# ExaScience/bpmf

Hardware: AMD Instinct MI355X
Metric: user+item column samples/sec per Gibbs iter; test RMSE vs reference (higher is better)
Workload: dtype f64

## Files before the change

bpmf_amd/csrc/kernels.h:

```cpp
#pragma once
#include <hip/hip_runtime.h>
#include <stdint.h>

#include "philox.h"
#include "args.h"

namespace bpmf {

typedef double d4 __attribute__((ext_vector_type(4)));

__device__ __forceinline__ d4 mfma16(double a, double b, d4 c)
{
    return __builtin_amdgcn_mfma_f64_16x16x4f64(a, b, c, 0, 0, 0);
}

__device__ __forceinline__ double mfma44(double a, double b, double c)
{
    return __builtin_amdgcn_mfma_f64_4x4x4f64(a, b, c, 0, 0, 0);
}

template <int K>
struct Rot44 {
    static constexpr int NT = K / 16;
    __host__ __device__ static constexpr int nrot(int TI, int TJ) { return TI == TJ ? 3 : 4; }
// ... 18 lines not shown
    const int lo = __builtin_amdgcn_update_dpp(0, (int)v, CTRL, 0xF, 0xF, true);
    const int hi = __builtin_amdgcn_update_dpp(0, (int)(v >> 32), CTRL, 0xF, 0xF, true);
    return __builtin_bit_cast(double, ((long long)hi << 32) | (unsigned int)lo);
}

template <int K>
__device__ __forceinline__ void rot44_contract(const double (&yy)[K / 16], double (&C)[Rot44<K>::NACC])
{
    using G = Rot44<K>;
    constexpr int NT = K / 16;
    double rot[NT][3];
#pragma unroll
    for (int t = 0; t < NT; ++t) {
        rot[t][0] = yy[t];
        rot[t][1] = quad_rot<1>(yy[t]);
        rot[t][2] = quad_rot<2>(yy[t]);
    }
#pragma unroll
    for (int TI = 0; TI < NT; ++TI)
#pragma unroll
        for (int TJ = TI; TJ < NT; ++TJ)
#pragma unroll
            for (int d = 0; d < G::nrot(TI, TJ); ++d) {
                if (d < 3) C[G::aoff(TI, TJ) + d] = mfma44(yy[TI], rot[TJ][d], C[G::aoff(TI, TJ) + d]);
                else C[G::aoff(TI, TJ) + d] = mfma44(rot[TI][1], yy[TJ], C[G::aoff(TI, TJ) + d]);
            }
}

template <int K, typename Sink>
__device__ __forceinline__ void rot44_images(const double (&C)[Rot44<K>::NACC], double *buf0, double *buf1, int lane, Sink &&sink)
{
    using G = Rot44<K>;
    constexpr int NT = G::NT;
    const int i = lane >> 4, b = (lane >> 2) & 3, j = lane & 3;
    int tix = 0;
#pragma unroll
    for (int TI = 0; TI < NT; ++TI)
#pragma unroll
        for (int TJ = TI; TJ < NT; ++TJ, ++tix) {
            double *img = (tix & 1) ? buf1 : buf0;
#pragma unroll
            for (int d = 0; d < G::nrot(TI, TJ); ++d) {
                const int row = d < 3 ? 4 * b + i : 4 * ((b + 1) & 3) + i, col = d < 3 ? 4 * ((b + d) & 3) + j : 4 * b + j;
                const double v = C[G::aoff(TI, TJ) + d];
                img[row * 16 + col] = v;
                if (TI == TJ && d > 0) img[col * 16 + row] = v;
            }
            __syncthreads();
#pragma unroll
            for (int m = 0; m < 4; ++m) sink(tix, TI, TJ, m, img[(4 * m + i) * 16 + (lane & 15)]);
            __syncthreads();
        }
}

__device__ __forceinline__ double rsqrt_nr(double d)
{
    const double y0 = __builtin_amdgcn_rsq(d);
    const double e = fma(-d, y0 * y0, 1.0);
    const double q = e * fma(0.375, e, 0.5);
    return fma(y0, q, y0);
}

__device__ __forceinline__ double gbcast(double v, int base_bytes, int off)
{
    const int lo = __builtin_amdgcn_ds_bpermute(base_bytes + 4 * off, __double2loint(v));
    const int hi = __builtin_amdgcn_ds_bpermute(base_bytes + 4 * off, __double2hiint(v));
    return __hiloint2double(hi, lo);
}

__device__ __forceinline__ double bcast(double v, int src)
{
    const int lo = __builtin_amdgcn_readlane(__double2loint(v), src);
    const int hi = __builtin_amdgcn_readlane(__double2hiint(v), src);
    return __hiloint2double(hi, lo);
}


__device__ __forceinline__ double polar_r2(double x, double y)
{
#pragma clang fp contract(off)
    return x * x + y * y;
}

__device__ __forceinline__ uint32_t sample_counter(int64_t idx, int ktrue, uint32_t iter_plus_1)
{
    return (uint32_t)((uint64_t)(idx + 1) * (uint64_t)ktrue * (uint64_t)iter_plus_1);
}

#define BPMF_RLX_SYSTEM_ __ATOMIC_RELAXED, __HIP_MEMORY_SCOPE_SYSTEM
enum { BPMF_TMO_GATE = 1, BPMF_TMO_PARAMS = 2, BPMF_TMO_STATS = 3 };
__device__ __forceinline__ void flag_timeout(unsigned long long *tmo, unsigned long long what)
{
    if (tmo) __hip_atomic_store(tmo, what, BPMF_RLX_SYSTEM_);
}

__device__ __forceinline__ void wait_params(const SampleArgs &a)
{
    if (a.gate_flag == nullptr) return;
    const unsigned long long t0 = wall_clock64();
    const unsigned long long limit = a.wait_ticks + (a.wait_ticks >> 1);
    while ((unsigned)__builtin_amdgcn_readfirstlane((int)__hip_atomic_load(a.gate_flag, __ATOMIC_RELAXED, __HIP_MEMORY_SCOPE_AGENT)) != a.gate_want) {
        __builtin_amdgcn_s_sleep(8);
        if (wall_clock64() - t0 > limit) {
            if (threadIdx.x == 0) flag_timeout(a.tmo, BPMF_TMO_PARAMS);
            break;
        }
    }
    asm volatile("" ::: "memory");
}

#ifndef BPMF_PROFILING
#define BPMF_PROFILING 0
#endif
constexpr bool kProfiling = BPMF_PROFILING != 0;
__device__ __forceinline__ uint32_t ablate_bits(const SampleArgs &a)
{
    if constexpr (kProfiling) return a.ablate;
    else return 0u;
}

__device__ __forceinline__ void stamp(const SampleArgs &a, int w, int slot)
{
    if constexpr (!kProfiling) {
        __builtin_amdgcn_sched_barrier(0);
        return;
    }
    if (a.stamps == nullptr || threadIdx.x != 0) return;
    const int probe = (w == 0) ? 0 : ((w == a.nwork / 2) ? 1 : -1);
    if (probe >= 0 && slot < 64) a.stamps[probe * 64 + slot] = wall_clock64();
}

__device__ __forceinline__ int rank_below(unsigned long long m)
{
    return (int)__builtin_amdgcn_mbcnt_hi((unsigned)(m >> 32), __builtin_amdgcn_mbcnt_lo((unsigned)m, 0u));
}

template <int NMAX>
__device__ __forceinline__ void draw_normals(uint32_t counter, int n, double *out_lds, int lane, int pad_to = 0)
{
    for (int i = n + lane; i < pad_to; i += 64) out_lds[i] = 0.0;
    int produced = 0;
    uint32_t base = 0;
    while (produced < n) {
        const Philox4 b = stream_block(counter, base + (uint32_t)lane);
        const double x = 2.0 * canonical53(b.w[3], b.w[2]) - 1.0;
        const double y = 2.0 * canonical53(b.w[1], b.w[0]) - 1.0;
        const double r2 = polar_r2(x, y);
        const bool acc = !(r2 > 1.0 || r2 == 0.0);
        const unsigned long long m = __ballot(acc);
        const int rank = produced + rank_below(m);
        if (acc && rank < n) {
            out_lds[rank] = y * polar_mult(r2);
        }
        produced += __popcll(m);
        base += 64u;
    }
}

template <int NMAX>
__device__ __forceinline__ void draw_normals_deferred(uint32_t counter, int n, double *out_lds, double *r2_lds, int lane, int pad_to = 0)
{
    for (int i = n + lane; i < pad_to; i += 64) out_lds[i] = 0.0;
    int produced = 0;
    uint32_t base = 0;
    while (produced < n) {
        const Philox4 b = stream_block(counter, base + (uint32_t)lane);
        const double x = 2.0 * canonical53(b.w[3], b.w[2]) - 1.0;
        const double y = 2.0 * canonical53(b.w[1], b.w[0]) - 1.0;
        const double r2 = polar_r2(x, y);
        const bool acc = !(r2 > 1.0 || r2 == 0.0);
        const unsigned long long m = __ballot(acc);
        const int rank = produced + rank_below(m);
        if (acc && rank < n) { out_lds[rank] = y; r2_lds[rank] = r2; }
        produced += __popcll(m);
        base += 64u;
    }
    for (int i = lane; i < n; i += 64) {
        const double r2 = r2_lds[i];
        out_lds[i] = out_lds[i] * polar_mult(r2);
    }
}

template <int NMAX>
__device__ __forceinline__ void draw_normals_pair(uint32_t counterA, uint32_t counterB, int n, double *outA, double *outB,
                                                  double *r2A, double *r2B, int lane, int pad_to = 0)
{
    for (int i = n + lane; i < pad_to; i += 64) { outA[i] = 0.0; outB[i] = 0.0; }
    auto attempt = [&](uint32_t counter, uint32_t block, double &y, double &r2) -> bool {
        const Philox4 b = stream_block(counter, block);
        const double x = 2.0 * canonical53(b.w[3], b.w[2]) - 1.0;
        y = 2.0 * canonical53(b.w[1], b.w[0]) - 1.0;
        r2 = polar_r2(x, y);
        return !(r2 > 1.0 || r2 == 0.0);
    };
    int prodA, prodB;
    {
        double y, r2;
        bool acc = attempt(counterA, (uint32_t)lane, y, r2);
        unsigned long long m = __ballot(acc);
        int rank = rank_below(m);
        if (acc && rank < n) { outA[rank] = y; r2A[rank] = r2; }
        prodA = __popcll(m);
        acc = attempt(counterB, (uint32_t)lane, y, r2);
        m = __ballot(acc);
        rank = rank_below(m);
        if (acc && rank < n) { outB[rank] = y; r2B[rank] = r2; }
        prodB = __popcll(m);
    }
    const bool hi = lane >= 32;
    const int l32 = lane & 31;
    uint32_t base = 64u;
    while (prodA < n || prodB < n) {
        double y, r2;
        const bool acc = attempt(hi ? counterB : counterA, base + (uint32_t)l32, y, r2);
        const unsigned long long m = __ballot(acc);
        const unsigned mA = (unsigned)m, mB = (unsigned)(m >> 32);
        const int rank = hi ? prodB + (int)__builtin_amdgcn_mbcnt_hi(mB, 0u) : prodA + (int)__builtin_amdgcn_mbcnt_lo(mA, 0u);
        if (acc && rank < n) { (hi ? outB : outA)[rank] = y; (hi ? r2B : r2A)[rank] = r2; }
        prodA += __popc(mA); prodB += __popc(mB);
        base += 32u;
    }
    for (int i = lane; i < n; i += 64) {
        const double ra = r2A[i], rb = r2B[i];
        outA[i] = outA[i] * polar_mult(ra);
        outB[i] = outB[i] * polar_mult(rb);
    }
}

template <int K>
__device__ __forceinline__ void gram_chunk(const int32_t *__restrict__ rowidx, const double *__restrict__ vals, int len,
                                           const double *__restrict__ other, const double *__restrict__ zero_row, double mean, double alpha,
                                           d4 (&acc)[Geo<K>::NTRI], double (&r)[Geo<K>::NT], int lane, int rowmask = -1)
{
    constexpr int NT = Geo<K>::NT;
    const int kq = lane >> 4, li = lane & 15;
    int ri_n = (0 + lane < len) ? rowidx[lane] : -1;
    double wv_n = (0 + lane < len) ? (vals[lane] - mean) * alpha : 0.0;
    for (int b = 0; b < len; b += 64) {
        const int ri = ri_n;
        const double wv = wv_n;
        if (b + 64 < len) {
            const int q = b + 64 + lane;
            ri_n = (q < len) ? rowidx[q] : -1;
            wv_n = (q < len) ? (vals[q] - mean) * alpha : 0.0;
        }
        const int nsteps = (len - b >= 64) ? 16 : (len - b + 3) >> 2;
        double y[4][NT], w[4];
        auto gather = [&](int g, double (&yy)[4][NT], double (&ww)[4]) {
#pragma unroll
            for (int s = 0; s < 4; ++s) {
                const int src = (g * 4 + s) * 4 + kq;
                const int row = __shfl(ri, src);
                ww[s] = __shfl(wv, src);
                const double *col = (row >= 0) ? other + (size_t)(row & rowmask) * K : zero_row;
#pragma unroll
                for (int t = 0; t < NT; ++t) yy[s][t] = col[(t * 16 + li < K) ? t * 16 + li : 0];
            }
        };
        gather(0, y, w);
#pragma unroll
        for (int g = 0; g < 4; ++g) {
            if (g * 4 >= nsteps) break;
            double yn[4][NT], wn[4];
            const bool more = (g + 1) * 4 < nsteps;
            if (g < 3 && more) gather(g + 1, yn, wn);
#pragma unroll
            for (int s = 0; s < 4; ++s) {
#pragma unroll
                for (int t = 0; t < NT; ++t) r[t] = fma(y[s][t], w[s], r[t]);
                int tri = 0;
#pragma unroll
                for (int I = 0; I < NT; ++I)
#pragma unroll
                    for (int J = I; J < NT; ++J, ++tri) acc[tri] = mfma16(y[s][I], y[s][J], acc[tri]);
            }
            if (g < 3 && more) {
#pragma unroll
                for (int s = 0; s < 4; ++s) {
                    w[s] = wn[s];
#pragma unroll
                    for (int t = 0; t < NT; ++t) y[s][t] = yn[s][t];
                }
            }
        }
    }
#pragma unroll
    for (int t = 0; t < NT; ++t) {
        r[t] += __shfl_xor(r[t], 16);
        r[t] += __shfl_xor(r[t], 32);
    }
}

template <int CTRL>
__device__ __forceinline__ double row_ror_add(double x)
{
    const long long v = __builtin_bit_cast(long long, x);
    const int lo = (int)v, hi = (int)(v >> 32);
    const int rlo = __builtin_amdgcn_update_dpp(0, lo, CTRL, 0xF, 0xF, true);
    const int rhi = __builtin_amdgcn_update_dpp(0, hi, CTRL, 0xF, 0xF, true);
    const long long rv = ((long long)rhi << 32) | (unsigned int)rlo;
    return x + __builtin_bit_cast(double, rv);
}

template <bool WT> struct IdxBlockT { int ri; double v; int base; };
template <> struct IdxBlockT<true> { int ri; double v; int base; double s; };
typedef IdxBlockT<false> IdxBlock;
template <bool WT = false>
__device__ __forceinline__ IdxBlockT<WT> load_idx_block(const int32_t *__restrict__ rowidx, const double *__restrict__ vals, int base, int lane, int len,
                                                        const double *__restrict__ safe, const double *__restrict__ sw = nullptr)
{
    IdxBlockT<WT> r;
    const int q = base + lane;
    const int32_t *pr = (q < len) ? rowidx + q : reinterpret_cast<const int32_t *>(safe);
    const double *pv = (q < len) ? vals + q : safe;
    r.ri = *pr;
    r.v = *pv;
    if constexpr (WT) {
        const double *ps = (q < len) ? sw + q : safe;
        r.s = *ps;
    }
    r.base = base;
    return r;
}

template <int K, bool WT = false>
__device__ __forceinline__ void gram_chunk44(const int32_t *__restrict__ rowidx, const double *__restrict__ vals, int len,
                                             const double *__restrict__ other, const double *__restrict__ zero_row,
                                             double mean, double alpha, IdxBlockT<WT> cur, IdxBlockT<WT> nxt,
                                             double (&acc)[Geo44<K>::NB], double (&rr)[Geo44<K>::NG], int lane, int rowmask = -1,
                                             const double *__restrict__ sw = nullptr)
{
    using G = Geo44<K>;
    constexpr int NG = G::NG, NL = G::NL;
    typedef double dd2 __attribute__((ext_vector_type(2)));
    const int slot = lane >> 2, x = lane & 3;
    auto gather = [&](const IdxBlockT<WT> &ib, int gg, dd2 (&yy)[NL], double &ww, double &ss) {
        const int src = gg * 16 + slot;
        const int row = __shfl(ib.ri, src);
        ww = (__shfl(ib.v, src) - mean) * alpha;
        if constexpr (WT) ss = __shfl(ib.s, src);
        const double *base = (ib.base + src < len) ? other + (size_t)(row & rowmask) * K : zero_row;
        const dd2 *p = reinterpret_cast<const dd2 *>(base + 2 * x);
#pragma unroll
        for (int h = 0; h < NL; ++h) yy[h] = p[4 * h];
    };
    auto contract = [&](const dd2 (&yy)[NL], double ww, double ss) {
        double R[NG];
#pragma unroll
        for (int h = 0; h < NL; ++h) { R[2 * h] = yy[h].x; R[2 * h + 1] = yy[h].y; }
        if constexpr (WT) {
#pragma unroll
            for (int g = 0; g < NG; ++g) R[g] *= ss;
        }
#pragma unroll
        for (int g = 0; g < NG; ++g) rr[g] = fma(R[g], ww, rr[g]);
        int blk = 0;
#pragma unroll
        for (int g = 0; g < NG; ++g)
#pragma unroll
            for (int g2 = g; g2 < NG; ++g2, ++blk) acc[blk] = mfma44(R[g], R[g2], acc[blk]);
    };
    if (len <= 0) return;
    dd2 yA[NL], yB[NL];
    double wA, wB = 0.0, sA = 0.0, sB = 0.0;
    gather(cur, 0, yA, wA, sA);
    int b0 = 0;
    for (; b0 + 64 < len; b0 += 64) {
        IdxBlockT<WT> nn{};
        if constexpr (!WT) nn = load_idx_block<WT>(rowidx, vals, b0 + 128, lane, len, zero_row, sw);
        gather(cur, 1, yB, wB, sB);
        contract(yA, wA, sA);
        gather(cur, 2, yA, wA, sA);
        contract(yB, wB, sB);
        gather(cur, 3, yB, wB, sB);
        contract(yA, wA, sA);
        gather(nxt, 0, yA, wA, sA);
        contract(yB, wB, sB);
        cur = nxt;
        if constexpr (WT) nxt = load_idx_block<WT>(rowidx, vals, b0 + 128, lane, len, zero_row, sw);
        else nxt = nn;
    }
    const int ng = (len - b0 + 15) >> 4;
    if (ng > 1) gather(cur, 1, yB, wB, sB);
    contract(yA, wA, sA);
    if (ng > 1) {
        if (ng > 2) gather(cur, 2, yA, wA, sA);
        contract(yB, wB, sB);
        if (ng > 2) {
            if (ng > 3) gather(cur, 3, yB, wB, sB);
            contract(yA, wA, sA);
            if (ng > 3) contract(yB, wB, sB);
        }
    }
}

typedef double gs_raw __attribute__((ext_vector_type(2)));
__device__ __forceinline__ gs_raw load_gs_rec(const GatherRec *__restrict__ rec, int g, unsigned slot_bytes)
{
    return *reinterpret_cast<const gs_raw *>(reinterpret_cast<const char *>(rec + 16 * g) + slot_bytes);
}

template <int K>
__device__ __forceinline__ void gram_stream44(const GatherRec *__restrict__ rec, int ng, const double *__restrict__ other,
                                              const double *__restrict__ zero_row, double alpha, gs_raw r0, gs_raw r1, unsigned slot_bytes,
                                              double (&acc)[Geo44<K>::NB], double (&rr)[Geo44<K>::NG], int lane)
{
    using G = Geo44<K>;
    constexpr int NG = G::NG, NL = G::NL;
    typedef double dd2 __attribute__((ext_vector_type(2)));
    const int x = lane & 3;
    const dd2 *ox = reinterpret_cast<const dd2 *>(other + 2 * x), *zx = reinterpret_cast<const dd2 *>(zero_row + 2 * x);
    auto gather = [&](const gs_raw &rc, dd2 (&yy)[NL], double &ww) {
        const int off = (int)__builtin_bit_cast(long long, rc.x);
        ww = rc.y * alpha;
        const dd2 *p = (off >= 0) ? ox + off : zx;
#pragma unroll
        for (int h = 0; h < NL; ++h) yy[h] = p[4 * h];
    };
    auto contract = [&](const dd2 (&yy)[NL], double ww) {
        double R[NG];
#pragma unroll
        for (int h = 0; h < NL; ++h) { R[2 * h] = yy[h].x; R[2 * h + 1] = yy[h].y; }
#pragma unroll
        for (int g = 0; g < NG; ++g) rr[g] = fma(R[g], ww, rr[g]);
        int blk = 0;
#pragma unroll
        for (int g = 0; g < NG; ++g)
#pragma unroll
            for (int g2 = g; g2 < NG; ++g2, ++blk) acc[blk] = mfma44(R[g], R[g2], acc[blk]);
    };
    if (ng <= 0) return;
    dd2 yA[NL], yB[NL];
    double wA, wB = 0.0;
    gather(r0, yA, wA);
    r0 = load_gs_rec(rec, 2, slot_bytes);
    if (ng > 1) gather(r1, yB, wB);
    r1 = load_gs_rec(rec, 3, slot_bytes);
    contract(yA, wA);
    int g = 1;
    for (; g + 2 < ng; g += 2) {
        gather(r0, yA, wA);
        r0 = load_gs_rec(rec, g + 3, slot_bytes);
        contract(yB, wB);
        gather(r1, yB, wB);
        r1 = load_gs_rec(rec, g + 4, slot_bytes);
        contract(yA, wA);
    }
    if (g < ng) {
        if (g + 1 < ng) gather(r0, yA, wA);
        contract(yB, wB);
        if (g + 1 < ng) contract(yA, wA);
    }
}

template <int K>
__device__ __forceinline__ void assemble44(double (&acc)[Geo44<K>::NB], double (&rr)[Geo44<K>::NG], double *sA, double *sb,
                                           int LD, int lane)
{
    using G = Geo44<K>;
    constexpr int NG = G::NG;
    static_assert(NG % 2 == 0, "block rows are written in pairs");
    const int i = lane >> 4, b = (lane >> 2) & 3, j = lane & 3;
    auto blk = [](int g, int g2) constexpr { return g * NG - (g * (g - 1)) / 2 + (g2 - g); };
    double *up = sA + (2 * i) * LD + 2 * j;
    double *lo = sA + (2 * j) * LD + 2 * i;
#pragma unroll
    for (int g = 0; g < NG; g += 2) {
#pragma unroll
        for (int t = blk(g, g); t < blk(g + 1, NG - 1) + 1; ++t) {
            const double v = row_ror_add<0x128>(acc[t]);
            acc[t] = row_ror_add<0x124>(v);
        }
        if (b == 0) {
            up[G::idx(g + 1, 0) * LD + G::idx(g + 1, 0)] = acc[blk(g + 1, g + 1)];
#pragma unroll
            for (int g2 = g; g2 < NG; g2 += 2) {
                double2 v; v.x = acc[blk(g, g2)]; v.y = acc[blk(g, g2 + 1)];
                *reinterpret_cast<double2 *>(&up[G::idx(g, 0) * LD + G::idx(g2, 0)]) = v;
                if (g2 > g) {
                    double2 w; w.x = acc[blk(g + 1, g2)]; w.y = acc[blk(g + 1, g2 + 1)];
                    *reinterpret_cast<double2 *>(&up[G::idx(g + 1, 0) * LD + G::idx(g2, 0)]) = w;
                }
            }
        } else if (b == 1) {
            lo[G::idx(g + 1, 0) * LD + G::idx(g, 0)] = acc[blk(g, g + 1)];
#pragma unroll
            for (int g2 = g + 2; g2 < NG; ++g2) {
                double2 v; v.x = acc[blk(g, g2)]; v.y = acc[blk(g + 1, g2)];
                *reinterpret_cast<double2 *>(&lo[G::idx(g2, 0) * LD + G::idx(g, 0)]) = v;
            }
        }
    }
#pragma unroll
    for (int g = 0; g < NG; ++g) {
        double v = row_ror_add<0x128>(rr[g]);
        v = row_ror_add<0x124>(v);
        v += __shfl_xor(v, 16);
        v += __shfl_xor(v, 32);
        if (lane < 4) sb[G::idx(g, lane)] = v;
    }
}

template <int K>
__device__ __forceinline__ void deposit_column(const SampleArgs &a, int64_t idx, const d4 (&acc)[Geo<K>::NTRI],
                                               const double (&r)[Geo<K>::NT], double *lds, int slot, int lane)
{
    using G = Geo<K>;
    constexpr int NT = G::NT;
    const int kq = lane >> 4, li = lane & 15;
    double *sL = lds + slot * G::SLOT, *sY = sL + G::PLEN, *sZ = sY + K;

    draw_normals<K>(sample_counter(idx, a.ktrue, a.iter_plus_1), a.ktrue, sZ, lane, K);
    const double *LF = a.prop_lambda ? a.prop_lambda + (size_t)(idx - a.col_from) * K * K : a.LambdaF;

    int tri = 0;
#pragma unroll
    for (int I = 0; I < NT; ++I)
#pragma unroll
        for (int J = I; J < NT; ++J, ++tri)
#pragma unroll
            for (int reg = 0; reg < 4; ++reg) {
                const int gi = I * 16 + kq + 4 * reg, gj = J * 16 + li;
                const int row = (I == J) ? gi : gj, col = (I == J) ? gj : gi;
                if (row < K && col <= row)
                    sL[tri_off(row) + col] = (a.diag_only && row != col) ? 0.0 : fma(a.alpha, acc[tri][reg], LF[row + col * K]);
            }
    if (kq == 0) {
#pragma unroll
        for (int t = 0; t < NT; ++t)
            if (t * 16 + li < K) {
                double lm = a.Lmu[t * 16 + li];
                if (a.prop_lambda) {
                    lm = 0.0;
                    for (int j = 0; j < K; ++j) lm = fma(LF[t * 16 + li + j * K], a.mu[j], lm);
                }
                sY[t * 16 + li] = lm + r[t];
            }
    }
    if (lane == 0) reinterpret_cast<long long *>(lds + G::C * G::SLOT)[slot] = idx;
}

template <int K>
struct Pivot { double dinv0, dinv1, l10; };

template <int K>
__device__ __forceinline__ Pivot<K> factor_block(double pa, double pb, double pc)
{
    Pivot<K> v;
    v.dinv0 = rsqrt_nr(pa);
    const double rdet = rsqrt_nr(fma(pa, pc, -(pb * pb)));
    v.dinv1 = rdet * (pa * v.dinv0);
    v.l10 = pb * v.dinv0;
    return v;
}

template <int K>
__device__ __forceinline__ void finish_slots(const SampleArgs &a, double *lds, int nfilled, int lane_in)
{
    using G = Geo<K>;
    constexpr int NP = G::NP;
    int lane = lane_in;
    asm volatile("" : "+v"(lane));
    const int c = lane / K, i = lane % K;
    double *sL = lds + c * G::SLOT, *sY = sL + G::PLEN, *sZ = sY + K;
    double *myrow = sL + tri_off(i);
    const int gbase = 4 * (c * K);
    __syncthreads();

    double row[K + 1];
#pragma unroll
    for (int j = 0; j < K; j += 2) {
        const double2 g = *reinterpret_cast<const double2 *>(&myrow[j]);
        row[j] = g.x;
        row[j + 1] = g.y;
    }
    row[K] = sY[i];
    const double zi = sZ[i];
    Pivot<K> pv = factor_block<K>(sL[0], sL[tri_off(1)], sL[tri_off(1) + 1]);
    __syncthreads();

#pragma unroll
    for (int p = 0; p < NP; ++p) {
        const int k = 2 * p;
        double2 lp;
        lp.x = row[k] * pv.dinv0;
        lp.y = fma(-lp.x, pv.l10, row[k + 1]) * pv.dinv1;
        if (i >= k) *reinterpret_cast<double2 *>(&myrow[k]) = lp;

        double na = 0.0, nb = 0.0, nc = 0.0;
        if (p + 1 < NP) {
            na = gbcast(row[k + 2], gbase, k + 2);
            nb = gbcast(row[k + 2], gbase, k + 3);
            nc = gbcast(row[k + 3], gbase, k + 3);
        }
        const double rb0 = gbcast(row[K], gbase, k), rb1 = gbcast(row[K], gbase, k + 1);
        __syncthreads();
        const double2 L = *reinterpret_cast<const double2 *>(&myrow[k]);
        Pivot<K> pn = pv;
        if (p + 1 < NP) {
            const double2 l0 = *reinterpret_cast<const double2 *>(&sL[tri_off(k + 2) + k]);
            const double2 l1 = *reinterpret_cast<const double2 *>(&sL[tri_off(k + 3) + k]);
            const double pa = fma(-l0.y, l0.y, fma(-l0.x, l0.x, na));
            const double pb = fma(-l1.y, l0.y, fma(-l1.x, l0.x, nb));
            const double pc = fma(-l1.y, l1.y, fma(-l1.x, l1.x, nc));
            pn = factor_block<K>(pa, pb, pc);
        }
        const double yk = rb0 * pv.dinv0;
        const double yk1 = fma(-pv.l10, yk, rb1) * pv.dinv1;
        if (i == 0) *reinterpret_cast<double2 *>(&sY[k]) = double2{yk, yk1};
        row[K] = fma(-L.y, yk1, fma(-L.x, yk, row[K]));
#pragma unroll
        for (int j = k + 2; j < K; ++j) {
            const double2 A = *reinterpret_cast<const double2 *>(&sL[tri_off(j) + k]);
            row[j] = fma(-L.y, A.y, fma(-L.x, A.x, row[j]));
        }
#pragma unroll
        for (int m = k + 2; m < K + 1; ++m) asm volatile("" : "+v"(row[m]));
        pv = pn;
    }
    __syncthreads();

    double bi = sY[i] + zi;
    const double my_dinv = 1.0 / myrow[i];
    constexpr int BB = K < 8 ? K : 8;
#pragma unroll
    for (int kb = K - BB; kb >= 0; kb -= BB) {
        double lv[BB];
#pragma unroll
        for (int t = 0; t < BB; ++t) lv[t] = sL[tri_off(kb + t) + i];
#pragma unroll
        for (int t = BB - 1; t >= 0; --t) {
            const int k = kb + t;
            if (k == 0) continue;
            const double xk = gbcast(bi * my_dinv, gbase, k);
            bi = (i < k) ? fma(-lv[t], xk, bi) : bi;
        }
    }
    const double xi = bi * my_dinv;

    if (c < nfilled) {
        const long long idx = reinterpret_cast<const long long *>(lds + G::C * G::SLOT)[c];
        a.items[(size_t)idx * K + i] = xi;
        if (!(fabs(xi) <= 1.79769313486231570815e+308)) atomicMin(a.fail, (unsigned long long)idx);
    }
    __syncthreads();
}

#define BPMF_RLX_AGENT __ATOMIC_RELAXED, __HIP_MEMORY_SCOPE_AGENT

template <int K>
struct Geo1 {
    static constexpr int S = (64 / K < K / 2) ? 64 / K : K / 2;
    static constexpr int NP = K / 2;
    static constexpr int QN = NP / S;
    static constexpr int M = 2 * QN;
    static constexpr int FLD = K + 2;
    static constexpr bool PACKED = K == 64;
    __host__ __device__ static constexpr int roff_c(int j) { return (j & 1) ? ((j + 1) * (j + 1)) / 2 : (j * (j + 2)) / 2; }
    static constexpr int AWORDS = PACKED ? roff_c(K) : K * FLD;
    static constexpr int LANES = K * S;
    static constexpr int LDS_WORDS = AWORDS + 4 * K + 2;
    static constexpr int WPS = K == 32 ? 3 : (K < 32 ? 4 : 2);
};

template <int K, typename Assemble>
__device__ __forceinline__ void finish_single(const SampleArgs &a, int col_local, double *lds, int lane_in, bool have_z,
                                              Assemble &&assemble)
{
    int lane = lane_in;
    using G = Geo1<K>;
    constexpr int LD = G::FLD, S = G::S, NP = G::NP, QN = G::QN, M = G::M;
    asm volatile("" : "+v"(lane));
    double *sA = lds, *sb = lds + G::AWORDS, *sz = sb + K, *sdummy = sz + K, *szero = sdummy + 2 * K;
    auto roff = [](int j) -> int {
        if constexpr (G::PACKED) return (j & 1) ? ((j + 1) * (j + 1)) >> 1 : (j * (j + 2)) >> 1;
        else return j * G::FLD;
    };
    const int64_t idx = a.col_from + col_local;

    if (!have_z) draw_normals<K>(sample_counter(idx, a.ktrue, a.iter_plus_1), a.ktrue, sz, lane, K);

    const int l = lane & (G::LANES - 1);
    const int h = l / K, i = l % K;
    const double *LF = a.prop_lambda ? a.prop_lambda + (size_t)col_local * K * K : a.LambdaF;
    constexpr bool PRELOAD = K <= 32;
    double lf[PRELOAD ? M : 2];
    if constexpr (PRELOAD) {
#pragma unroll
        for (int q = 0; q < QN; ++q) {
            const int j = 2 * (q * S + h);
            lf[2 * q] = LF[i + j * K];
            lf[2 * q + 1] = LF[i + (j + 1) * K];
        }
    }
    double lmu = a.Lmu[i];
    if (a.prop_lambda) {
        lmu = 0.0;
        for (int j = 0; j < K; ++j) lmu = fma(LF[i + j * K], a.mu[j], lmu);
    }

    assemble(sA, sb, LD, lane);
    if (lane < 2) szero[lane] = 0.0;
    __syncthreads();

    double row[M + 2];
#pragma unroll
    for (int q = 0; q < QN; ++q) {
        double2 g;
        if constexpr (G::PACKED) {
            const int j = 2 * (q * S + h);
            g.x = sA[(j <= i) ? roff(i) + j : roff(j) + i];
            g.y = sA[(j + 1 <= i) ? roff(i) + j + 1 : roff(j + 1) + i];
        } else {
            g = *reinterpret_cast<const double2 *>(&sA[i * LD + 2 * (q * S + h)]);
        }
        if constexpr (PRELOAD) {
            row[2 * q] = fma(a.alpha, g.x, lf[2 * q]);
            row[2 * q + 1] = fma(a.alpha, g.y, lf[2 * q + 1]);
        } else {
            const int j = 2 * (q * S + h);
            row[2 * q] = fma(a.alpha, g.x, LF[i + j * K]);
            row[2 * q + 1] = fma(a.alpha, g.y, LF[i + (j + 1) * K]);
        }
    }
    if (a.diag_only) {
#pragma unroll
        for (int q = 0; q < QN; ++q) {
            const int j = 2 * (q * S + h);
            row[2 * q] = (j == i) ? row[2 * q] : 0.0;
            row[2 * q + 1] = (j + 1 == i) ? row[2 * q + 1] : 0.0;
        }
    }
    row[M] = (h == 0) ? lmu + sb[i] : 0.0;
    row[M + 1] = 0.0;
    const double zi = sz[i];
    double yi = 0.0;
    __syncthreads();

#pragma unroll
    for (int p = 0; p < NP; ++p) {
        const int hk = p % S, qk = p / S, k = 2 * p;
        const int src0 = hk * K + k, src1 = src0 + 1;
        const double pa = bcast(row[2 * qk], src0);
        const double pb = bcast(row[2 * qk], src1);
        const double pc = bcast(row[2 * qk + 1], src1);
        const double bk = bcast(row[M], k), bk1 = bcast(row[M], k + 1);
        const double dinv0 = rsqrt_nr(pa);
        const double rdet = rsqrt_nr(fma(pa, pc, -(pb * pb)));
        const double dinv1 = rdet * (pa * dinv0);
        const double l10 = pb * dinv0;
        const double yk = bk * dinv0;
        const double yk1 = fma(-l10, yk, bk1) * dinv1;
        yi = (i == k) ? yk : yi;
        yi = (i == k + 1) ? yk1 : yi;
        double2 lp;
        lp.x = row[2 * qk] * dinv0;
        lp.y = fma(-lp.x, l10, row[2 * qk + 1]) * dinv1;
        double *dst = (h == hk && (!G::PACKED || i >= k)) ? &sA[roff(i) + k] : &sdummy[2 * i];
        *reinterpret_cast<double2 *>(dst) = lp;
        __syncthreads();
        const double2 L = *reinterpret_cast<const double2 *>((!G::PACKED || i >= k) ? &sA[roff(i) + k] : szero);
        row[M] = fma(-L.y, yk1, fma(-L.x, yk, row[M]));
        if constexpr (S > 1) {
            const int j0 = 2 * (qk * S + h);
            const double2 A0 = *reinterpret_cast<const double2 *>(&sA[roff(j0) + k]);
            const double2 A1 = *reinterpret_cast<const double2 *>(&sA[roff(j0 + 1) + k]);
            const double u0 = fma(-L.y, A0.y, fma(-L.x, A0.x, row[2 * qk]));
            const double u1 = fma(-L.y, A1.y, fma(-L.x, A1.x, row[2 * qk + 1]));
            row[2 * qk] = (h > hk) ? u0 : row[2 * qk];
            row[2 * qk + 1] = (h > hk) ? u1 : row[2 * qk + 1];
        }
#pragma unroll
        for (int q = qk + 1; q < QN; ++q) {
            const int j0 = 2 * (q * S + h);
            const double2 A0 = *reinterpret_cast<const double2 *>(&sA[roff(j0) + k]);
            const double2 A1 = *reinterpret_cast<const double2 *>(&sA[roff(j0 + 1) + k]);
            row[2 * q] = fma(-L.y, A0.y, fma(-L.x, A0.x, row[2 * q]));
            row[2 * q + 1] = fma(-L.y, A1.y, fma(-L.x, A1.x, row[2 * q + 1]));
        }
#pragma unroll
        for (int m = 2 * qk; m < M + 1; ++m) asm volatile("" : "+v"(row[m]));
    }

    double bi = yi + zi;
    const double my_dinv = 1.0 / sA[roff(i) + i];
    constexpr int BB = K < 8 ? K : 8;
#pragma unroll
    for (int kb = K - BB; kb >= 0; kb -= BB) {
        double lv[BB];
#pragma unroll
        for (int t = 0; t < BB; ++t) lv[t] = *((i < kb + t) ? &sA[roff(kb + t) + i] : szero);
#pragma unroll
        for (int t = BB - 1; t >= 0; --t) {
            const int k = kb + t;
            if (k == 0) continue;
            const double xk = bcast(bi * my_dinv, k);
            bi = fma(-lv[t], xk, bi);
        }
    }
    const double xi = bi * my_dinv;

    if (lane < K) a.items[(size_t)idx * K + lane] = xi;
    const bool bad = !(fabs(xi) <= 1.79769313486231570815e+308);
    if (__any(bad) && lane == 0) atomicMin(a.fail, (unsigned long long)idx);
}

template <int K>
__device__ __forceinline__ void colstats_body(int w, const double *__restrict__ items, int64_t c0, int64_t c1, int nwaves,
                                              double *partials, const unsigned long long *__restrict__ fail_in,
                                              double *__restrict__ out, unsigned *ticket, unsigned *flag, unsigned seq,
                                              unsigned long long *tmo, unsigned long long wait_ticks, double *img);
__device__ __forceinline__ void gate_stage_body(int block, int nblocks, const unsigned *gate_host, unsigned want, const double *src_host,
                                                double *__restrict__ dst, int n, unsigned *dflag, unsigned dval,
                                                unsigned long long *tmo, unsigned long long wait_ticks);

template <int K, bool GS, bool WT = false>
__device__ __forceinline__ void sample1_body(const SampleArgs &a, const FusedArgs &f, double *lds)
{
    const int lane = threadIdx.x;
    int bid = blockIdx.x;
    if (f.gate_host) {
        if (bid == 0) { gate_stage_body(0, 1, f.gate_host, f.gate_want, f.src_host, f.dst, f.n, f.dflag, f.dval, a.tmo, a.wait_ticks); return; }
        --bid;
    }
    if (bid < f.nstat) {
        colstats_body<K>(bid, f.st_items, f.st_c0, f.st_c1, f.nstat, f.st_partials, f.st_fail, f.st_out, f.st_ticket, f.st_flag, f.st_seq,
                         f.st_tmo, a.wait_ticks, lds);
        return;
    }
    const int w = bid - f.nstat;
    const int col = a.wi_col[w];
    const int64_t p0 = a.wi_p0[w];
    const int len = a.wi_len[w];
    const int mc = a.wi_mc[w];

    const int glen = (ablate_bits(a) & 2u) ? 0 : len;
    static_assert(!(GS && WT), "the gather stream carries no weights");
    IdxBlockT<WT> ib0{}, ib1{};
    gs_raw gr0{}, gr1{};
    const GatherRec *rec = nullptr;
    const unsigned slot_bytes = 16u * ((unsigned)lane >> 2);
    int ng = 0;
    if constexpr (GS) {
        rec = a.gs_rec + (size_t)a.gs_g0[w] * 16;
        ng = (ablate_bits(a) & 2u) ? 0 : a.gs_ng[w];
        gr0 = load_gs_rec(rec, 0, slot_bytes);
        gr1 = load_gs_rec(rec, 1, slot_bytes);
    } else {
        ib0 = load_idx_block<WT>(a.rowidx + p0, a.vals + p0, 0, lane, glen, a.zero_row, WT ? a.sw + p0 : nullptr);
        ib1 = load_idx_block<WT>(a.rowidx + p0, a.vals + p0, 64, lane, glen, a.zero_row, WT ? a.sw + p0 : nullptr);
    }

    if (mc < 0 && !(ablate_bits(a) & 1u))
        draw_normals<K>(sample_counter(a.col_from + col, a.ktrue, a.iter_plus_1), a.ktrue, lds + Geo1<K>::AWORDS + K, lane, K);

    static_assert(K <= 32, "k_sample1: K <= 32 (K = 64 runs the slab form, K = 128 the workgroup form)");
    {
        using G4 = Geo44<K>;
        constexpr int NB = G4::NB, NG = G4::NG, PART = G4::PART;
        double acc[NB], rr[NG];
#pragma unroll
        for (int t = 0; t < NB; ++t) acc[t] = 0.0;
#pragma unroll
        for (int t = 0; t < NG; ++t) rr[t] = 0.0;
        if constexpr (GS)
            gram_stream44<K>(rec, ng, a.other_items, a.zero_row, a.alpha, gr0, gr1, slot_bytes, acc, rr, lane);
        else
            gram_chunk44<K, WT>(a.rowidx + p0, a.vals + p0, glen, a.other_items, a.zero_row, a.mean_rating, a.alpha, ib0, ib1, acc, rr, lane,
                                (ablate_bits(a) & 4u) ? 63 : -1, WT ? a.sw + p0 : nullptr);
        if (ablate_bits(a) & 1u) {
            double v = rr[0];
#pragma unroll
            for (int t = 0; t < NB; ++t) v += acc[t];
            if (mc < 0 && lane < K) a.items[(size_t)(a.col_from + col) * K + lane] = v;
            return;
        }
        if (mc >= 0) {
            const int nch = a.mc_nchunks[mc];
            double *pbase = a.partials + (size_t)a.mc_slot0[mc] * PART;
            double *p = pbase + (size_t)a.wi_chunk[w] * PART;
#pragma unroll
            for (int t = 0; t < NB; ++t) __hip_atomic_store(&p[t * 64 + lane], acc[t], BPMF_RLX_AGENT);
#pragma unroll
            for (int t = 0; t < NG; ++t) __hip_atomic_store(&p[(NB + t) * 64 + lane], rr[t], BPMF_RLX_AGENT);
            asm volatile("s_waitcnt vmcnt(0)" ::: "memory");
            unsigned t = 0;
            if (lane == 0) t = __hip_atomic_fetch_add(&a.mc_count[mc], 1u, BPMF_RLX_AGENT);
            t = __builtin_amdgcn_readfirstlane(t);
            if ((int)t != nch - 1) return;
            if (lane == 0) __hip_atomic_store(&a.mc_count[mc], 0u, BPMF_RLX_AGENT);
#pragma unroll
            for (int t2 = 0; t2 < NB; ++t2) acc[t2] = 0.0;
#pragma unroll
            for (int t2 = 0; t2 < NG; ++t2) rr[t2] = 0.0;
            for (int ch = 0; ch < nch; ++ch) {
                const double *pc = pbase + (size_t)ch * PART;
                double tmp[NB + NG];
#pragma unroll
                for (int t2 = 0; t2 < NB + NG; ++t2) tmp[t2] = __hip_atomic_load(&pc[t2 * 64 + lane], BPMF_RLX_AGENT);
#pragma unroll
                for (int t2 = 0; t2 < NB; ++t2) acc[t2] += tmp[t2];
#pragma unroll
                for (int t2 = 0; t2 < NG; ++t2) rr[t2] += tmp[NB + t2];
            }
        }
        wait_params(a);
        finish_single<K>(a, col, lds, lane, mc < 0,
                         [&](double *sA, double *sb, int LD, int ln) { assemble44<K>(acc, rr, sA, sb, LD, ln); });
    }
}

template <int K>
__global__ __launch_bounds__(64, Geo1<K>::WPS) void k_sample1(SampleArgs a, FusedArgs f)
{
    __shared__ __attribute__((aligned(16))) double lds[Geo1<K>::LDS_WORDS];
    sample1_body<K, true>(a, f, lds);
}

template <int K>
__global__ __launch_bounds__(64, Geo1<K>::WPS) void k_sample1i(SampleArgs a, FusedArgs f)
{
    __shared__ __attribute__((aligned(16))) double lds[Geo1<K>::LDS_WORDS];
    sample1_body<K, false>(a, f, lds);
}

template <int K>
__global__ __launch_bounds__(64, Geo1<K>::WPS) void k_sample1w(SampleArgs a, FusedArgs f)
{
    __shared__ __attribute__((aligned(16))) double lds[Geo1<K>::LDS_WORDS];
    sample1_body<K, false, true>(a, f, lds);
}

#define BPMF_RLX_SYSTEM __ATOMIC_RELAXED, __HIP_MEMORY_SCOPE_SYSTEM
__device__ __forceinline__ void publish_when_last(unsigned *ticket, unsigned nblocks, unsigned *flag_host, unsigned seq,
                                                  unsigned *rearm = nullptr, unsigned *rearm2 = nullptr)
{
    asm volatile("s_waitcnt vmcnt(0)" ::: "memory");
    __syncthreads();
    if (threadIdx.x == 0) {
        const unsigned t = __hip_atomic_fetch_add(ticket, 1u, BPMF_RLX_AGENT);
        if (t == nblocks - 1) {
            __hip_atomic_store(ticket, 0u, BPMF_RLX_AGENT);
            if (rearm) __hip_atomic_store(rearm, 0u, BPMF_RLX_AGENT);
            if (rearm2) __hip_atomic_store(rearm2, 0u, BPMF_RLX_AGENT);
            __hip_atomic_store(flag_host, seq, BPMF_RLX_SYSTEM);
        }
    }
}

template <int K>
constexpr bool kColstatsRot = (K == 64);

template <int K>
__device__ __forceinline__ void colstats_accumulate(const double *__restrict__ items, int64_t b, int64_t e,
                                                    d4 (&acc)[Geo<K>::NTRI], double (&r)[Geo<K>::NT], int lane, double *img,
                                                    const int32_t *__restrict__ list = nullptr, int64_t c0 = 0)
{
    constexpr int NT = Geo<K>::NT;
    constexpr bool ROT = kColstatsRot<K>;
    const int kq = lane >> 4, li = lane & 15;
    double C[ROT ? Rot44<K>::NACC : 1];
#pragma unroll
    for (int t = 0; t < (ROT ? Rot44<K>::NACC : 1); ++t) C[t] = 0.0;
#pragma unroll
    for (int t = 0; t < Geo<K>::NTRI; ++t) acc[t] = d4{0.0, 0.0, 0.0, 0.0};
#pragma unroll
    for (int t = 0; t < NT; ++t) r[t] = 0.0;
    double yn[2][NT];
    int64_t idn[2];
    auto ids = [&](int64_t c, int64_t (&id)[2]) {
#pragma unroll
        for (int s = 0; s < 2; ++s) {
            const int64_t pos = (c + s * 4 + kq < e) ? c + s * 4 + kq : b;
            id[s] = list ? c0 + (int64_t)list[pos] : pos;
        }
    };
    auto fetch = [&](const int64_t (&id)[2], double (&yy)[2][NT]) {
#pragma unroll
        for (int s = 0; s < 2; ++s) {
            const double *x = items + (size_t)id[s] * K;
#pragma unroll
            for (int t = 0; t < NT; ++t) yy[s][t] = x[(t * 16 + li < K) ? t * 16 + li : 0];
        }
    };
    if (b < e) {
        int64_t id0[2];
        ids(b, id0);
        fetch(id0, yn);
        ids((b + 8 < e) ? b + 8 : b, idn);
    }
    for (int64_t c = b; c < e; c += 8) {
        double y[2][NT];
#pragma unroll
        for (int s = 0; s < 2; ++s) {
            const bool ok = c + s * 4 + kq < e;
#pragma unroll
            for (int t = 0; t < NT; ++t) y[s][t] = (ok && (t * 16 + li < K)) ? yn[s][t] : 0.0;
        }
        fetch(idn, yn);
        ids((c + 16 < e) ? c + 16 : b, idn);
#pragma unroll
        for (int s = 0; s < 2; ++s) {
#pragma unroll
            for (int t = 0; t < NT; ++t) r[t] += y[s][t];
            if constexpr (ROT) {
                rot44_contract<K>(y[s], C);
            } else {
                int tri = 0;
#pragma unroll
                for (int I = 0; I < NT; ++I)
#pragma unroll
                    for (int J = I; J < NT; ++J, ++tri) acc[tri] = mfma16(y[s][I], y[s][J], acc[tri]);
            }
        }
    }
    if constexpr (ROT) rot44_images<K>(C, img, img + 256, lane, [&](int tix, int, int, int m, double v) { acc[tix][m] = v; });
#pragma unroll
    for (int t = 0; t < NT; ++t) {
        r[t] += __shfl_xor(r[t], 16);
        r[t] += __shfl_xor(r[t], 32);
    }
}

template <int K>
__device__ __forceinline__ void colstats_body(int w, const double *__restrict__ items, int64_t c0, int64_t c1, int nwaves,
                                              double *partials, const unsigned long long *__restrict__ fail_in,
                                              double *__restrict__ out, unsigned *ticket, unsigned *flag, unsigned seq,
                                              unsigned long long *tmo, unsigned long long wait_ticks, double *img)
{
    constexpr int NT = Geo<K>::NT, NTRI = Geo<K>::NTRI, PART = Geo<K>::PART;
    constexpr int NSUMS = blob::res_sums(K), NSLICE = (NSUMS + 15) / 16, FAILD = blob::res_failD(K), FAIL = blob::res_fail(K);
    const int lane = threadIdx.x;
    const int64_t n = c1 - c0;
    const int64_t per = (((n + nwaves - 1) / nwaves) + 3) & ~(int64_t)3;
    const int64_t b = c0 + w * per;
    const int64_t e = (b + per < c1) ? b + per : c1;

    {
        d4 acc[NTRI];
        double r[NT];
        colstats_accumulate<K>(items, b, e, acc, r, lane, img);
        double *p = partials + (size_t)w * PART;
#pragma unroll
        for (int t = 0; t < NTRI; ++t)
#pragma unroll
            for (int reg = 0; reg < 4; ++reg) __hip_atomic_store(&p[(t * 4 + reg) * 64 + lane], acc[t][reg], BPMF_RLX_AGENT);
        if (lane < 16) {
#pragma unroll
            for (int t = 0; t < NT; ++t) __hip_atomic_store(&p[NTRI * 256 + t * 16 + lane], r[t], BPMF_RLX_AGENT);
        }
    }

    const int nfin = nwaves < NSLICE ? nwaves : NSLICE;
    asm volatile("s_waitcnt vmcnt(0)" ::: "memory");
    unsigned tk = 0;
    if (lane == 0) tk = __hip_atomic_fetch_add(ticket, 1u, BPMF_RLX_AGENT);
    tk = __builtin_amdgcn_readfirstlane(tk);
    if ((int)tk < nwaves - nfin) return;
    const int f = (int)tk - (nwaves - nfin);
    if (lane == 0) {
        const unsigned long long t0 = wall_clock64();
        while (__hip_atomic_load(ticket, BPMF_RLX_AGENT) < (unsigned)nwaves) {
            __builtin_amdgcn_s_sleep(1);
            if (wait_ticks && wall_clock64() - t0 > wait_ticks) { flag_timeout(tmo, BPMF_TMO_STATS); break; }
        }
    }
    __syncthreads();

    const int o = lane & 15, grp = lane >> 4;
    for (int slice = f; slice < NSLICE; slice += nfin) {
        const int eo = slice * 16 + o;
        double s = 0.0;
        if (eo < NSUMS) {
            int off;
            if (eo < K * K) {
                int i = eo % K, j = eo / K;
                if (i > j) { const int t = i; i = j; j = t; }
                const int I = i >> 4, J = j >> 4;
                const int tri = I * NT - (I * (I - 1)) / 2 + (J - I);
                const int ii = i & 15, jj = j & 15;
                off = (tri * 4 + (ii >> 2)) * 64 + (ii & 3) * 16 + jj;
            } else {
                off = NTRI * 256 + (eo - K * K);
            }
            const int pw = (nwaves + 3) >> 2;
            const int w0 = grp * pw, w1 = (w0 + pw < nwaves) ? w0 + pw : nwaves;
            double acc[16];
#pragma unroll
            for (int u = 0; u < 16; ++u) acc[u] = 0.0;
            for (int ww = w0; ww < w1; ww += 16) {
                double v[16];
#pragma unroll
                for (int u = 0; u < 16; ++u)
                    v[u] = __hip_atomic_load(&partials[(size_t)((ww + u < w1) ? ww + u : w0) * PART + off], BPMF_RLX_AGENT);
#pragma unroll
                for (int u = 0; u < 16; ++u) acc[u] += (ww + u < w1) ? v[u] : 0.0;
            }
#pragma unroll
            for (int h = 8; h >= 1; h >>= 1)
#pragma unroll
// ... 341 lines not shown
```

Measured before the change: 105.5 million.

## Use permlane swaps for rhs reduction and restructure single-column Cholesky solve

Replaces the shfl_xor butterfly in the rhs reduction with v_permlane16/32_swap, pairing groups so that each swap reduces two values at once and fewer cross-lane ops are issued. In the single-column Cholesky path, y values go to a small LDS array instead of per-lane selects, and the dummy-store redirect becomes a predicated store. The back-substitution for the non-packed layout now preloads the whole column, pins the loaded values in registers and guards the update by lane. The trade-offs are extra LDS traffic for y, predicated branches, and reliance on permlane swap intrinsics that exist only on newer CDNA targets.

```diff
diff --git a/bpmf_amd/csrc/kernels.h b/bpmf_amd/csrc/kernels.h
--- a/bpmf_amd/csrc/kernels.h
+++ b/bpmf_amd/csrc/kernels.h
@@ -344,6 +344,25 @@
     return x + __builtin_bit_cast(double, rv);
 }
 
+template <int W>
+__device__ __forceinline__ double2 lane_swap(double a, double b)
+{
+    static_assert(W == 16 || W == 32, "v_permlane16_swap or v_permlane32_swap");
+    const unsigned alo = (unsigned)__double2loint(a), ahi = (unsigned)__double2hiint(a);
+    const unsigned blo = (unsigned)__double2loint(b), bhi = (unsigned)__double2hiint(b);
+    unsigned xlo, xhi, ylo, yhi;
+    if constexpr (W == 16) {
+        const auto lo = __builtin_amdgcn_permlane16_swap(alo, blo, false, false);
+        const auto hi = __builtin_amdgcn_permlane16_swap(ahi, bhi, false, false);
+        xlo = lo[0]; ylo = lo[1]; xhi = hi[0]; yhi = hi[1];
+    } else {
+        const auto lo = __builtin_amdgcn_permlane32_swap(alo, blo, false, false);
+        const auto hi = __builtin_amdgcn_permlane32_swap(ahi, bhi, false, false);
+        xlo = lo[0]; ylo = lo[1]; xhi = hi[0]; yhi = hi[1];
+    }
+    return double2{__hiloint2double((int)xhi, (int)xlo), __hiloint2double((int)yhi, (int)ylo)};
+}
+
 template <bool WT> struct IdxBlockT { int ri; double v; int base; };
 template <> struct IdxBlockT<true> { int ri; double v; int base; double s; };
 typedef IdxBlockT<false> IdxBlock;
@@ -533,13 +552,26 @@
             }
         }
     }
+    static_assert(NG == 2 || NG % 4 == 0, "the rhs butterfly takes two or a multiple of four groups");
 #pragma unroll
     for (int g = 0; g < NG; ++g) {
-        double v = row_ror_add<0x128>(rr[g]);
-        v = row_ror_add<0x124>(v);
-        v += __shfl_xor(v, 16);
-        v += __shfl_xor(v, 32);
-        if (lane < 4) sb[G::idx(g, lane)] = v;
+        const double v = row_ror_add<0x128>(rr[g]);
+        rr[g] = row_ror_add<0x124>(v);
+    }
+#pragma unroll
+    for (int g = 0; g < NG; g += 2) {
+        const double2 s = lane_swap<16>(rr[g], rr[g + 1]);
+        rr[g >> 1] = s.x + s.y;
+    }
+    constexpr int NQ = (NG + 3) / 4;
+#pragma unroll
+    for (int m = 0; m < NQ; ++m) {
+        const double2 s = lane_swap<32>(rr[2 * m], rr[NG == 2 ? 0 : 2 * m + 1]);
+        rr[m] = s.x + s.y;
+    }
+    if (b == 0) {
+#pragma unroll
+        for (int m = 0; m < NQ; ++m) sb[G::idx(NG == 2 ? (i & 1) : 4 * m + i, j)] = rr[m];
     }
 }
 
@@ -701,7 +733,7 @@
     __host__ __device__ static constexpr int roff_c(int j) { return (j & 1) ? ((j + 1) * (j + 1)) / 2 : (j * (j + 2)) / 2; }
     static constexpr int AWORDS = PACKED ? roff_c(K) : K * FLD;
     static constexpr int LANES = K * S;
-    static constexpr int LDS_WORDS = AWORDS + 4 * K + 2;
+    static constexpr int LDS_WORDS = AWORDS + 3 * K + 2;
     static constexpr int WPS = K == 32 ? 3 : (K < 32 ? 4 : 2);
 };
 
@@ -713,7 +745,7 @@
     using G = Geo1<K>;
     constexpr int LD = G::FLD, S = G::S, NP = G::NP, QN = G::QN, M = G::M;
     asm volatile("" : "+v"(lane));
-    double *sA = lds, *sb = lds + G::AWORDS, *sz = sb + K, *sdummy = sz + K, *szero = sdummy + 2 * K;
+    double *sA = lds, *sb = lds + G::AWORDS, *sz = sb + K, *sy = sz + K, *szero = sy + K;
     auto roff = [](int j) -> int {
         if constexpr (G::PACKED) return (j & 1) ? ((j + 1) * (j + 1)) >> 1 : (j * (j + 2)) >> 1;
         else return j * G::FLD;
@@ -742,7 +774,7 @@
     }
 
     assemble(sA, sb, LD, lane);
-    if (lane < 2) szero[lane] = 0.0;
+    if constexpr (G::PACKED) { if (lane < 2) szero[lane] = 0.0; }
     __syncthreads();
 
     double row[M + 2];
@@ -776,7 +808,6 @@
     row[M] = (h == 0) ? lmu + sb[i] : 0.0;
     row[M + 1] = 0.0;
     const double zi = sz[i];
-    double yi = 0.0;
     __syncthreads();
 
 #pragma unroll
@@ -793,13 +824,12 @@
         const double l10 = pb * dinv0;
         const double yk = bk * dinv0;
         const double yk1 = fma(-l10, yk, bk1) * dinv1;
-        yi = (i == k) ? yk : yi;
-        yi = (i == k + 1) ? yk1 : yi;
+        if (lane == 0) *reinterpret_cast<double2 *>(&sy[k]) = double2{yk, yk1};
         double2 lp;
         lp.x = row[2 * qk] * dinv0;
         lp.y = fma(-lp.x, l10, row[2 * qk + 1]) * dinv1;
-        double *dst = (h == hk && (!G::PACKED || i >= k)) ? &sA[roff(i) + k] : &sdummy[2 * i];
-        *reinterpret_cast<double2 *>(dst) = lp;
+        if (h == hk && (!G::PACKED || i >= k))
+            *reinterpret_cast<double2 *>(&sA[roff(i) + k]) = lp;
         __syncthreads();
         const double2 L = *reinterpret_cast<const double2 *>((!G::PACKED || i >= k) ? &sA[roff(i) + k] : szero);
         row[M] = fma(-L.y, yk1, fma(-L.x, yk, row[M]));
@@ -824,20 +854,35 @@
         for (int m = 2 * qk; m < M + 1; ++m) asm volatile("" : "+v"(row[m]));
     }
 
-    double bi = yi + zi;
+    double bi = sy[i] + zi;
     const double my_dinv = 1.0 / sA[roff(i) + i];
-    constexpr int BB = K < 8 ? K : 8;
+    constexpr int BB = G::PACKED ? 8 : K;
 #pragma unroll
     for (int kb = K - BB; kb >= 0; kb -= BB) {
         double lv[BB];
 #pragma unroll
-        for (int t = 0; t < BB; ++t) lv[t] = *((i < kb + t) ? &sA[roff(kb + t) + i] : szero);
+        for (int t = 0; t < BB; ++t) {
+            if constexpr (G::PACKED) lv[t] = *((i < kb + t) ? &sA[roff(kb + t) + i] : szero);
+            else lv[t] = sA[roff(kb + t) + i];
+        }
+        if constexpr (!G::PACKED) {
+            static_assert(BB % 8 == 0, "the pins take eight values each");
+#pragma unroll
+            for (int t = 0; t < BB; t += 8)
+                asm volatile("" : "+v"(lv[t]), "+v"(lv[t + 1]), "+v"(lv[t + 2]), "+v"(lv[t + 3]), "+v"(lv[t + 4]), "+v"(lv[t + 5]),
+                             "+v"(lv[t + 6]), "+v"(lv[t + 7]));
+        }
 #pragma unroll
         for (int t = BB - 1; t >= 0; --t) {
             const int k = kb + t;
             if (k == 0) continue;
             const double xk = bcast(bi * my_dinv, k);
-            bi = fma(-lv[t], xk, bi);
+            if constexpr (G::PACKED) {
+                bi = fma(-lv[t], xk, bi);
+            } else if (i < k) {
+                bi = fma(-lv[t], xk, bi);
+                __builtin_amdgcn_sched_barrier(0);
+            }
         }
     }
     const double xi = bi * my_dinv;
```

Result: no change. 105.3 million (-0.2%).
